# leotimus/binary-recommendation

Measured on AMD Instinct MI355X. Metric: (user,item) pairs/sec at batch 65536 dim 64, higher is better.
Workload: dtype f32; 1 GPU; NeuMF-A full training step (trainers/NFC_plain.py graph: 4 embeddings, 128->100->50->10->1, BCE, Keras-Adam adam_dense), embed_dim=64, 1000000 users x 100000 items per GPU, batch 65536 per GPU, uniform ids; global_batch=65536, parallelism=single GPU, steps_per_graph_launch=4, optimizer=adam_dense (deferred replay)

## Files before the change

### binary-recommendation_amd/csrc/dense_fwd.hip

```cpp
#include "common.h"
#include <stdlib.h>
#include "philox.h"
#include "dense.h"
#include "stamps.h"

namespace br {

using f32x4 = __attribute__((ext_vector_type(4))) float;

constexpr int kRep = BR_STAT_REPLICAS;
#ifdef BR_ABLATE_MFMA
#define BR_ABLATE_KEEP(c) (c)
#else
#define BR_ABLATE_KEEP(c) true
#endif

__device__ __forceinline__ f32x4 mfma16(float a, float b, f32x4 c) {
  return __builtin_amdgcn_mfma_f32_16x16x4f32(a, b, c, 0, 0, 0);
}


__global__ __launch_bounds__(256) void keep_bits_kernel(KeepArgs a) {
  dropout_resolve(a.drop);
  keep_bits_block(a, (int)blockIdx.y, (int64_t)blockIdx.x);
}

struct FwdArgs {
  const float* x; int64_t ldx;
  const float* W; const float* bias;
  float* y; int64_t ldy;
  int64_t batch;
  int K, N, act;
  const float* scale; const float* shift;
  brBnFold bn;
  const uint32_t* keep; int kw;
  float inv_keep;
  double* stats;
  const float* yin;
};

__device__ __forceinline__ float keep_if(float x, uint32_t w, uint32_t pos) {
  const int m = __builtin_amdgcn_sbfe((int)w, pos, 1u);
  return __int_as_float(__float_as_int(x) & m);
}

__device__ __forceinline__ float act_fwd(float z, int sigmask, float floor_) {
  const float s = __builtin_amdgcn_rcpf(1.0f + __builtin_amdgcn_exp2f(z * -1.44269504088896340736f));
  const float m = fmaxf(z, floor_);
  return __int_as_float((__float_as_int(s) & sigmask) | (__float_as_int(m) & ~sigmask));
}

template <int KJ, bool VEC>
__device__ __forceinline__ void fwd_load_tile(float4 (&av)[KJ], uint32_t (&kb)[(KJ + 1) / 2], const FwdArgs& a, int64_t tile, int c16, int g) {
  int64_t arow = (tile << 4) + c16;
  arow = arow < a.batch ? arow : a.batch - 1;
  const float* p = a.x + arow * a.ldx + 4 * g;
  const int klast = 16 * (KJ - 1) + 4 * g;
  if (VEC) {
#pragma unroll
    for (int j = 0; j < KJ - 1; ++j) av[j] = *reinterpret_cast<const float4*>(p + 16 * j);
    av[KJ - 1] = *reinterpret_cast<const float4*>(klast < a.K ? p + 16 * (KJ - 1) : p - 4 * g);
  } else {
#pragma unroll
    for (int j = 0; j < KJ - 1; ++j) av[j] = make_float4(p[16 * j], p[16 * j + 1], p[16 * j + 2], p[16 * j + 3]);
    const float* q = p - 4 * g;
    const int K1 = a.K - 1;
    av[KJ - 1] = make_float4(q[klast < K1 ? klast : K1], q[klast + 1 < K1 ? klast + 1 : K1], q[klast + 2 < K1 ? klast + 2 : K1], q[klast + 3 < K1 ? klast + 3 : K1]);
  }
  if (a.keep) {
    const uint32_t* kr = a.keep + arow * a.kw;
#pragma unroll
    for (int w = 0; w < (KJ + 1) / 2; ++w) kb[w] = kr[w];
  }
}

constexpr int kPatchLd = 20;

template <bool VEC>
__device__ __forceinline__ void fwd_epilogue(const f32x4& acc, const FwdArgs& a, float* patch, float* yrow, int64_t rbase, int nt, int c16, int g,
                                             const int (&vmask)[4], bool row_ok, float bv, int sigmask, float floor_, float& ssum, float& ssq) {
  const int n = nt * 16 + c16;
  const bool last = nt * 16 + 16 > a.N;
  const int cmask = (!last || n < a.N) ? -1 : 0;
  float yv[4] = {0.f, 0.f, 0.f, 0.f};
  if (a.yin) {
#pragma unroll
    for (int r = 0; r < 4; ++r) yv[r] = a.yin[(rbase + (vmask[r] ? 4 * g + r : 0)) * a.ldy + (cmask ? n : 0)];
  }
#pragma unroll
  for (int r = 0; r < 4; ++r) {
    const float z = fmaf(acc[r], a.inv_keep, bv) + yv[r];
    const float v = __int_as_float(__float_as_int(act_fwd(z, sigmask, floor_)) & vmask[r] & cmask);
    ssum += v;
    ssq = fmaf(v, v, ssq);
    patch[(4 * g + r) * kPatchLd + c16] = v;
  }
  __builtin_amdgcn_wave_barrier();
  const float4 o = *reinterpret_cast<const float4*>(patch + c16 * kPatchLd + 4 * g);
  __builtin_amdgcn_wave_barrier();
  float* dst = yrow + nt * 16;
  const int n0 = nt * 16 + 4 * g;
  if (VEC) {
    if (row_ok && (!last || n0 < a.N)) *reinterpret_cast<float4*>(dst) = o;
  } else if (row_ok) {
    if (n0 + 0 < a.N) dst[0] = o.x;
    if (n0 + 1 < a.N) dst[1] = o.y;
    if (n0 + 2 < a.N) dst[2] = o.z;
    if (n0 + 3 < a.N) dst[3] = o.w;
  }
}

template <bool VEC, int WN, int NT>
__device__ __forceinline__ void fwd_epilogue_multi(const f32x4 (&acc)[4], const FwdArgs& a, float* patch4, float* yrow, int64_t rbase, int nt0, int c16, int g,
                                                   const int (&vmask)[4], bool row_ok, const float* bs, int sigmask, float floor_, float (&ssum)[NT], float (&ssq)[NT]) {
#pragma unroll
  for (int w = 0; w < WN; ++w) {
    const int nt = nt0 + w, n = nt * 16 + c16;
    const bool last = nt * 16 + 16 > a.N;
    const int cmask = (!last || n < a.N) ? -1 : 0;
    const float bv = bs[n];
    float* patch = patch4 + w * 16 * kPatchLd;
#pragma unroll
    for (int r = 0; r < 4; ++r) {
      float z = fmaf(acc[w][r], a.inv_keep, bv);
      if (a.yin) z += a.yin[(rbase + (vmask[r] ? 4 * g + r : 0)) * a.ldy + (cmask ? n : 0)];
      const float v = __int_as_float(__float_as_int(act_fwd(z, sigmask, floor_)) & vmask[r] & cmask);
      ssum[nt] += v;
      ssq[nt] = fmaf(v, v, ssq[nt]);
      patch[(4 * g + r) * kPatchLd + c16] = v;
    }
  }
  __builtin_amdgcn_wave_barrier();
  const float* pr = patch4 + c16 * kPatchLd + 4 * g;
  const float4 z4 = make_float4(0.f, 0.f, 0.f, 0.f);
  const float4 o0 = *reinterpret_cast<const float4*>(pr);
  const float4 o1 = WN > 1 ? *reinterpret_cast<const float4*>(pr + 1 * 16 * kPatchLd) : z4;
  const float4 o2 = WN > 2 ? *reinterpret_cast<const float4*>(pr + 2 * 16 * kPatchLd) : z4;
  const float4 o3 = WN > 3 ? *reinterpret_cast<const float4*>(pr + 3 * 16 * kPatchLd) : z4;
  auto put = [&](const float4& o, int w) {
    const int nt = nt0 + w, n0 = nt * 16 + 4 * g;
    float* dst = yrow + nt * 16;
    if (VEC) {
      if (n0 < a.N) *reinterpret_cast<float4*>(dst) = o;
    } else {
      if (n0 + 0 < a.N) dst[0] = o.x;
      if (n0 + 1 < a.N) dst[1] = o.y;
      if (n0 + 2 < a.N) dst[2] = o.z;
      if (n0 + 3 < a.N) dst[3] = o.w;
    }
  };
  if (row_ok) {
    put(o0, 0);
    if (WN > 1) put(o1, 1);
    if (WN > 2) put(o2, 2);
    if (WN > 3) put(o3, 3);
  }
}

template <int NT, int KJ, bool VEC, int WPS, bool EMU>
__global__ __launch_bounds__(256 * WPS, WPS) void dense_fwd_kernel(const FwdArgs a) {
  extern __shared__ __attribute__((aligned(16))) float smem[];
  constexpr int kFwdThreads = 256 * WPS, kFwdWaves = 4 * WPS;
  constexpr int Np = NT * 16, Kp = KJ * 16, KWJ = (KJ + 1) / 2;
  constexpr int KB = (KJ + 1) / 2;
  constexpr int kWsFloats = EMU ? KB * 3 * 4 * Np * 4 : Kp * Np;
  float* Ws = smem;
  float* ssb = Ws + kWsFloats;
  float* bs = ssb + 2 * Kp;
  float* patches = bs + Np;
  constexpr int kPatchesPerWave = WPS == 2 ? 4 : 1;
  float* redw = patches + kFwdWaves * kPatchesPerWave * 16 * kPatchLd;
  const int lane = threadIdx.x & 63, wave = threadIdx.x >> 6;
  const int c16 = lane & 15, g = lane >> 4;
  const int K = a.K, N = a.N;
  const int64_t batch = a.batch;
  const int64_t n_tiles = (batch + 15) >> 4;
  const int64_t tstride = (int64_t)gridDim.x * kFwdWaves;
  {
    const int slot = __builtin_amdgcn_readfirstlane(wave >> 2);
    if (slot == 0) __builtin_amdgcn_s_setprio(3);
    else if (slot == 1) __builtin_amdgcn_s_setprio(2);
    else if (slot == 2) __builtin_amdgcn_s_setprio(1);
  }

  BR_STAMP_DECL;
  BR_STAMP_RT(10);
  BR_STAMP(0);
  const bool wquad = EMU && (N & 3) == 0;
  constexpr int NQ = Np / 4, TOTQ = KB * 4 * NQ, TRQ = EMU ? (TOTQ + kFwdThreads - 1) / kFwdThreads : 1;
  constexpr int TOTS = KB * 4 * Np, TRS = EMU ? (TOTS + kFwdThreads - 1) / kFwdThreads : 1;
  float4 wq[TRQ][8];
  float wv1[TRS][8];
  if constexpr (EMU) {
    if (wquad) {
#pragma unroll
      for (int i = 0; i < TRQ; ++i) {
        const int idx = threadIdx.x + i * kFwdThreads;
        const int idc = idx < TOTQ ? idx : 0;
        const int Jg = idc / NQ, n = (idc - Jg * NQ) * 4;
        const int J = Jg >> 2, gg = Jg & 3;
        const int nc = n < N ? n : 0;
#pragma unroll
        for (int q = 0; q < 8; ++q) {
          const int k = 32 * J + 16 * (q >> 2) + 4 * gg + (q & 3);
          wq[i][q] = *reinterpret_cast<const float4*>(a.W + (int64_t)(k < K ? k : 0) * N + nc);
        }
      }
    } else {
#pragma unroll
      for (int i = 0; i < TRS; ++i) {
        const int idx = threadIdx.x + i * kFwdThreads;
        const int idc = idx < TOTS ? idx : 0;
        const int Jg = idc / Np, n = idc - Jg * Np;
        const int J = Jg >> 2, gg = Jg & 3;
        const int nc = n < N ? n : N - 1;
#pragma unroll
        for (int q = 0; q < 8; ++q) {
          const int k = 32 * J + 16 * (q >> 2) + 4 * gg + (q & 3);
          wv1[i][q] = a.W[(k < K ? k : K - 1) * N + nc];
        }
      }
    }
  }
  float4 av[KJ];
  uint32_t kb[KWJ];
  int64_t tile = (int64_t)blockIdx.x * kFwdWaves + wave;
  fwd_load_tile<KJ, VEC>(av, kb, a, tile, c16, g);
  BR_STAMP(1);

  if (wquad) {
#pragma unroll
    for (int i = 0; i < TRQ; ++i) {
      const int idx = threadIdx.x + i * kFwdThreads;
      const int Jg = idx / NQ, n = (idx - Jg * NQ) * 4;
      const int J = Jg >> 2, gg = Jg & 3;
      const int nin = n < N ? -1 : 0;
      uint32_t* wsu = reinterpret_cast<uint32_t*>(Ws);
#pragma unroll
      for (int e = 0; e < 4; ++e) {
        uint32_t ph[4], pm[4], pl[4];
#pragma unroll
        for (int q = 0; q < 4; ++q) {
          const int k0 = 32 * J + 16 * (q >> 1) + 4 * gg + 2 * (q & 1);
          const float4 v0 = wq[i][2 * q], v1 = wq[i][2 * q + 1];
          const float f0 = e == 0 ? v0.x : (e == 1 ? v0.y : (e == 2 ? v0.z : v0.w)), f1 = e == 0 ? v1.x : (e == 1 ? v1.y : (e == 2 ? v1.z : v1.w));
          split3(__int_as_float(__float_as_int(f0) & nin & (k0 < K ? -1 : 0)), __int_as_float(__float_as_int(f1) & nin & (k0 + 1 < K ? -1 : 0)), ph[q], pm[q], pl[q]);
        }
        if (idx < TOTQ) {
          *reinterpret_cast<uint4*>(wsu + ((((J * 3 + 0) * 4 + gg) * Np + n + e) << 2)) = make_uint4(ph[0], ph[1], ph[2], ph[3]);
          *reinterpret_cast<uint4*>(wsu + ((((J * 3 + 1) * 4 + gg) * Np + n + e) << 2)) = make_uint4(pm[0], pm[1], pm[2], pm[3]);
          *reinterpret_cast<uint4*>(wsu + ((((J * 3 + 2) * 4 + gg) * Np + n + e) << 2)) = make_uint4(pl[0], pl[1], pl[2], pl[3]);
        }
      }
      __builtin_amdgcn_sched_barrier(0);
    }
  } else if constexpr (EMU) {
    constexpr int TOT = TOTS, TR = TRS;
    auto& wv = wv1;
#pragma unroll
    for (int i = 0; i < TR; ++i) {
      const int idx = threadIdx.x + i * kFwdThreads;
      const int Jg = idx / Np, n = idx - Jg * Np;
      const int J = Jg >> 2, gg = Jg & 3;
      uint32_t ph[4], pm[4], pl[4];
#pragma unroll
      for (int q = 0; q < 4; ++q) {
        const int k0 = 32 * J + 16 * (q >> 1) + 4 * gg + 2 * (q & 1);
        const float w0 = (n < N && k0 < K) ? wv[i][2 * q] : 0.f, w1 = (n < N && k0 + 1 < K) ? wv[i][2 * q + 1] : 0.f;
        split3(w0, w1, ph[q], pm[q], pl[q]);
      }
      if (idx < TOT) {
        uint32_t* wsu = reinterpret_cast<uint32_t*>(Ws);
        *reinterpret_cast<uint4*>(wsu + ((((J * 3 + 0) * 4 + gg) * Np + n) << 2)) = make_uint4(ph[0], ph[1], ph[2], ph[3]);
        *reinterpret_cast<uint4*>(wsu + ((((J * 3 + 1) * 4 + gg) * Np + n) << 2)) = make_uint4(pm[0], pm[1], pm[2], pm[3]);
        *reinterpret_cast<uint4*>(wsu + ((((J * 3 + 2) * 4 + gg) * Np + n) << 2)) = make_uint4(pl[0], pl[1], pl[2], pl[3]);
      }
      __builtin_amdgcn_sched_barrier(0);
    }
  } else
  {
    constexpr int TOT = KJ * 4 * Np, TR = (TOT + kFwdThreads - 1) / kFwdThreads;
    float wv[TR][4];
#pragma unroll
    for (int i = 0; i < TR; ++i) {
      const int idx = threadIdx.x + i * kFwdThreads;
      const int idc = idx < TOT ? idx : 0;
      const int jg = idc / Np, n = idc - jg * Np;
      const int k0 = 4 * jg;
      const int nc = n < N ? n : N - 1;
#pragma unroll
      for (int q = 0; q < 4; ++q) wv[i][q] = a.W[(k0 + q < K ? k0 + q : K - 1) * N + nc];
    }
#pragma unroll
    for (int i = 0; i < TR; ++i) {
      const int idx = threadIdx.x + i * kFwdThreads;
      const int jg = idx / Np, n = idx - jg * Np;
      const int k0 = 4 * jg;
      const bool nin = n < N;
      if (idx < TOT)
        *reinterpret_cast<float4*>(Ws + idx * 4) = make_float4((nin && k0 + 0 < K) ? wv[i][0] : 0.f, (nin && k0 + 1 < K) ? wv[i][1] : 0.f,
                                                                (nin && k0 + 2 < K) ? wv[i][2] : 0.f, (nin && k0 + 3 < K) ? wv[i][3] : 0.f);
    }
  }
  for (int k = threadIdx.x; k < Kp; k += kFwdThreads) {
    float sc = k < K ? 1.f : 0.f, sh = 0.f;
    if (k < K && a.bn.stats) {
      double s1 = 0.0, s2 = 0.0;
      for (int r = 0; r < kRep; ++r) { s1 += a.bn.stats[(size_t)r * 2 * K + k]; s2 += a.bn.stats[(size_t)r * 2 * K + K + k]; }
      const double mu = s1 / a.bn.batch_total;
      double var = s2 / a.bn.batch_total - mu * mu;
      if (var < 0.0) var = 0.0;
      const float muf = (float)mu, varf = (float)var;
      const float rs = 1.0f / sqrtf(varf + a.bn.eps);
      sc = a.bn.gamma[k] * rs;
      sh = a.bn.beta[k] - muf * sc;
      if (blockIdx.x == 0) {
        a.bn.scale[k] = sc; a.bn.shift[k] = sh; a.bn.mean[k] = muf; a.bn.rstd[k] = rs;
        if (a.bn.moving_mean) {
          a.bn.moving_mean[k] = a.bn.moving_mean[k] * a.bn.momentum + muf * (1.0f - a.bn.momentum);
          a.bn.moving_var[k] = a.bn.moving_var[k] * a.bn.momentum + varf * (1.0f - a.bn.momentum);
        }
      }
    } else if (k < K && a.scale) { sc = a.scale[k]; sh = a.shift[k]; }
    ssb[k] = sc;
    ssb[Kp + k] = sh;
  }
  for (int n = threadIdx.x; n < Np; n += kFwdThreads) bs[n] = (a.bias && n < N) ? a.bias[n] : 0.f;
  BR_STAMP(2);
  __syncthreads();
  BR_STAMP(3);

  float* patch = patches + wave * kPatchesPerWave * 16 * kPatchLd;
  float ssum[NT], ssq[NT];
#pragma unroll
  for (int nt = 0; nt < NT; ++nt) { ssum[nt] = 0.f; ssq[nt] = 0.f; }
  const int sigmask = a.act == BR_ACT_SIGMOID ? -1 : 0;
  const float floor_ = a.act == BR_ACT_RELU ? 0.f : -__builtin_inff();

  while (tile < n_tiles) {
    const int64_t rbase = tile << 4;
    const bool affine = a.scale || a.bn.stats || 16 * KJ != K;
    if (VEC && (K & 3)) {
      const int klast = 16 * (KJ - 1) + 4 * g;
      if (klast + 1 >= K) av[KJ - 1].y = 0.f;
      if (klast + 2 >= K) av[KJ - 1].z = 0.f;
      if (klast + 3 >= K) av[KJ - 1].w = 0.f;
    }
#pragma unroll
    for (int j = 0; j < KJ; ++j) {
      if (affine) {
        const int k = 16 * j + 4 * g;
        const float4 sc = *reinterpret_cast<const float4*>(ssb + k), sh = *reinterpret_cast<const float4*>(ssb + Kp + k);
        av[j].x = av[j].x * sc.x + sh.x; av[j].y = av[j].y * sc.y + sh.y; av[j].z = av[j].z * sc.z + sh.z; av[j].w = av[j].w * sc.w + sh.w;
      }
      if (a.keep) {
        const uint32_t w = kb[j >> 1], p0 = 16u * (j & 1) + 4u * g;
        av[j].x = keep_if(av[j].x, w, p0); av[j].y = keep_if(av[j].y, w, p0 + 1);
        av[j].z = keep_if(av[j].z, w, p0 + 2); av[j].w = keep_if(av[j].w, w, p0 + 3);
      }
      __builtin_amdgcn_sched_barrier(0);
    }
    BR_STAMP(4);
    const int64_t left = batch - rbase;
    const int rows_left16 = left > 16 ? 16 : (int)left;
    int vmask[4];
#pragma unroll
    for (int r = 0; r < 4; ++r) vmask[r] = (4 * g + r < rows_left16) ? -1 : 0;
    const bool row_ok = c16 < rows_left16;
    float* yrow = a.y + (rbase + (row_ok ? c16 : 0)) * a.ldy + 4 * g;
    float4 avn[WPS == 2 ? KJ : 1];
    uint32_t kbn[WPS == 2 ? KWJ : 1];
    const bool has_next = tile + tstride < n_tiles;
    if (WPS == 2 && has_next) fwd_load_tile<KJ, VEC>(reinterpret_cast<float4 (&)[KJ]>(avn), reinterpret_cast<uint32_t (&)[KWJ]>(kbn), a, tile + tstride, c16, g);
    constexpr bool PRESPLIT = EMU && WPS == 2;
    uint32_t ah[PRESPLIT ? KB : 1][4], am[PRESPLIT ? KB : 1][4], al[PRESPLIT ? KB : 1][4];
    auto split_block = [&](int J, uint32_t (&h)[4], uint32_t (&m)[4], uint32_t (&l)[4]) {
      const int j1 = 2 * J + 1 < KJ ? 2 * J + 1 : 0;
      split3(av[2 * J].x, av[2 * J].y, h[0], m[0], l[0]);
      split3(av[2 * J].z, av[2 * J].w, h[1], m[1], l[1]);
      if (2 * J + 1 < KJ) {
        split3(av[j1].x, av[j1].y, h[2], m[2], l[2]);
        split3(av[j1].z, av[j1].w, h[3], m[3], l[3]);
      } else {
        h[2] = h[3] = m[2] = m[3] = l[2] = l[3] = 0u;
      }
    };
    if constexpr (PRESPLIT) {
#pragma unroll
      for (int J = 0; J < KB; ++J) {
        split_block(J, ah[J], am[J], al[J]);
        __builtin_amdgcn_sched_barrier(0);
// ... 101 lines not shown
      }
    }
  }
  BR_STAMP(9);
  BR_STAMP_RT(11);
  BR_STAMP_FLUSH(blockIdx.x * kFwdWaves + wave);
}

}

using namespace br;

static inline int tiles16(int v) { return (v + 15) / 16; }
constexpr int kMaxT = 8;

extern "C" int64_t brDropoutKeepWords(int64_t batch, int K) { return (batch > 0 ? batch : 0) * (int64_t)((K + 31) / 32); }

extern "C" int brDropoutKeepBits(float drop_p, uint64_t seed, uint32_t step, int64_t row0, int64_t batch, int n_sites, const uint32_t* sites,
                                 const int* widths, uint32_t* const* out, brStream stream) {
  return br::dropout_keep_bits_ahead(drop_p, seed, step, 0, row0, batch, n_sites, sites, widths, out, stream);
}

int br::make_keep_args(KeepArgs& a, float drop_p, uint64_t seed, uint32_t step, uint32_t step_add, int64_t row0, int64_t batch, int n_sites,
                       const uint32_t* sites, const int* widths, uint32_t* const* out) {
  BR_CHECK_ARG(n_sites >= 1 && n_sites <= 3 && sites && widths && out && batch >= 0, "brDropoutKeepBits: bad args (1..3 sites)");
  BR_CHECK_ARG(drop_p > 0.f && drop_p < 1.f, "brDropoutKeepBits: drop_p must be in (0,1)");
  a.n_sites = n_sites;
  for (int i = 0; i < 3; ++i) {
    const int j = i < n_sites ? i : 0;
    BR_CHECK_ARG(widths[j] >= 1 && out[j], "brDropoutKeepBits: bad site %d", j);
    a.s[i].out = out[j]; a.s[i].K = widths[j]; a.s[i].kw = (widths[j] + 31) / 32; a.s[i].site = sites[j];
  }
  a.drop = make_dropout(drop_p, seed, step, 0);
  if (const StepStateDev* ss = current_step_state()) a.drop.step_ptr = &ss->step;
  a.drop.step_add = step_add;
  a.row0 = row0; a.batch = batch;
  return BR_OK;
}

int br::dropout_keep_bits_ahead(float drop_p, uint64_t seed, uint32_t step, uint32_t step_add, int64_t row0, int64_t batch, int n_sites,
                                const uint32_t* sites, const int* widths, uint32_t* const* out, brStream stream) {
  KeepArgs a;
  const int rc = make_keep_args(a, drop_p, seed, step, step_add, row0, batch, n_sites, sites, widths, out);
  if (rc != BR_OK) return rc;
  if (batch == 0) return BR_OK;
  int kwmax = 0;
  for (int i = 0; i < n_sites; ++i) kwmax = a.s[i].kw > kwmax ? a.s[i].kw : kwmax;
  const dim3 grid((unsigned)ceil_div(batch * kwmax, 256), (unsigned)n_sites);
  keep_bits_kernel<<<grid, 256, 0, (hipStream_t)stream>>>(a);
  BR_CHECK_LAUNCH("brDropoutKeepBits");
  return BR_OK;
}

template <int NT, int KJ, bool VEC, int WPS, bool EMU>
static void launch_fwd_v(unsigned grid, size_t shmem, hipStream_t s, const FwdArgs& a) {
  static bool attr_set = false;
  if (!attr_set) {
    (void)hipFuncSetAttribute((const void*)dense_fwd_kernel<NT, KJ, VEC, WPS, EMU>, hipFuncAttributeMaxDynamicSharedMemorySize, 150 * 1024);
    attr_set = true;
  }
  dense_fwd_kernel<NT, KJ, VEC, WPS, EMU><<<grid, 256 * WPS, shmem, s>>>(a);
}
static int fwd_wps(int64_t batch, bool vec, int KJ, int NT, bool emu) {
  static const int forced = [] { const char* e = getenv("BR_FWD_WPS"); return e ? atoi(e) : 0; }();
  if (!vec) return 4;
  if (forced == 2 || forced == 4) return forced;
  if (emu && KJ >= 5 && NT >= 3 && NT != 4) return 2;
  return (KJ >= 8 && ceil_div(batch, (int64_t)16) >= (int64_t)2 * 256 * 8) ? 2 : 4;
}

template <int NT, int KJ>
static void launch_fwd(size_t shmem_words_fixed, int Np, hipStream_t s, const FwdArgs& a, bool emu) {
  const bool vec = (a.ldx % 4 == 0) && ((reinterpret_cast<uintptr_t>(a.x) & 15) == 0) && (a.ldy % 4 == 0) && ((reinterpret_cast<uintptr_t>(a.y) & 15) == 0) &&
                   (a.yin == nullptr || a.K % 4 == 0);
  const int wps = fwd_wps(a.batch, vec, KJ, NT, emu);
  const int waves = 4 * wps;
  const size_t shmem = (shmem_words_fixed + (size_t)waves * (wps == 2 ? 4 : 1) * 16 * kPatchLd + (size_t)waves * 2 * Np) * sizeof(float);
  const int64_t wgs = ceil_div(ceil_div(a.batch, (int64_t)16), (int64_t)waves);
  const unsigned grid = (unsigned)(wgs < 1 ? 1 : (wgs > 256 ? 256 : wgs));
  if (emu) {
    if (vec && wps == 2) launch_fwd_v<NT, KJ, true, 2, true>(grid, shmem, s, a);
    else if (vec) launch_fwd_v<NT, KJ, true, 4, true>(grid, shmem, s, a);
    else launch_fwd_v<NT, KJ, false, 4, true>(grid, shmem, s, a);
    return;
  }
  if (vec && wps == 2) launch_fwd_v<NT, KJ, true, 2, false>(grid, shmem, s, a);
  else if (vec) launch_fwd_v<NT, KJ, true, 4, false>(grid, shmem, s, a);
  else launch_fwd_v<NT, KJ, false, 4, false>(grid, shmem, s, a);
}

static int dense_forward_one(FwdArgs a, hipStream_t s) {
  const int NT = tiles16(a.N), KJ = tiles16(a.K), Kp = KJ * 16, Np = NT * 16;
  const bool emu = br::mlp_bf16x6();
  const size_t wimg = emu ? (size_t)((KJ + 1) / 2) * 3 * 4 * Np * 4 : (size_t)Kp * Np;
  const size_t fixed = wimg + 2 * (size_t)Kp + (size_t)Np;
#define BR_FWD_KJ(NTv, KJv) case KJv: launch_fwd<NTv, KJv>(fixed, Np, s, a, emu); break;
#define BR_FWD(NTv)                                                                                        \
  case NTv:                                                                                                \
    switch (KJ) { BR_FWD_KJ(NTv, 1) BR_FWD_KJ(NTv, 2) BR_FWD_KJ(NTv, 3) BR_FWD_KJ(NTv, 4) BR_FWD_KJ(NTv, 5) \
                  BR_FWD_KJ(NTv, 6) BR_FWD_KJ(NTv, 7) BR_FWD_KJ(NTv, 8) default: break; }                  \
    break;
  switch (NT) {
    BR_FWD(1) BR_FWD(2) BR_FWD(3) BR_FWD(4) BR_FWD(5) BR_FWD(6) BR_FWD(7) BR_FWD(8)
    default: br::set_error("brDenseForward: unsupported N"); return BR_ERR_UNSUPPORTED;
  }
  BR_CHECK_LAUNCH("brDenseForward");
  return BR_OK;
}

static inline int split_k(int K) { return ((K / 2 + 31) / 32) * 32; }

extern "C" int brDenseForward(const float* x, int64_t ldx, const float* W, const float* bias, float* y, int64_t ldy,
                              int64_t batch, int K, int N, int act, const float* in_scale, const float* in_shift,
                              const brBnFold* in_bn, float drop_p, const uint32_t* keep, double* stats, brStream stream) {
  BR_CHECK_ARG(x && W && y && batch >= 0 && K >= 1 && N >= 1, "brDenseForward: bad args");
  BR_CHECK_ARG(K <= 2 * kMaxT * 16 && N <= kMaxT * 16, "brDenseForward: K=%d N=%d exceed %d / %d", K, N, 2 * kMaxT * 16, kMaxT * 16);
  BR_CHECK_ARG(ldx >= K && ldy >= N, "brDenseForward: bad leading dims");
  BR_CHECK_ARG((in_scale == nullptr) == (in_shift == nullptr), "brDenseForward: in_scale/in_shift both or neither");
  BR_CHECK_ARG(!in_bn || (!in_scale && in_bn->stats && in_bn->gamma && in_bn->beta && in_bn->scale && in_bn->shift && in_bn->mean && in_bn->rstd &&
                          in_bn->batch_total > 0 && (in_bn->moving_mean == nullptr) == (in_bn->moving_var == nullptr) && K <= kMaxT * 16),
               "brDenseForward: in_bn needs stats, gamma, beta and the four outputs, no in_scale/in_shift, K <= %d", kMaxT * 16);
  BR_CHECK_ARG(drop_p >= 0.f && drop_p < 1.f, "brDenseForward: drop_p out of [0,1)");
  BR_CHECK_ARG((drop_p > 0.f) == (keep != nullptr), "brDenseForward: keep bits (brDropoutKeepBits) are required exactly when drop_p > 0");
  if (batch == 0) return BR_OK;
  hipStream_t s = (hipStream_t)stream;
  const int kw = (K + 31) / 32;
  brBnFold nofold{};
  FwdArgs a{x, ldx, W, bias, y, ldy, batch, K, N, act, in_scale, in_shift, in_bn ? *in_bn : nofold, keep, kw, drop_p > 0.f ? 1.0f / (1.0f - drop_p) : 1.0f, stats, nullptr};
  if (K <= kMaxT * 16) return dense_forward_one(a, s);
  const int Ka = split_k(K);
  FwdArgs h = a;
  h.K = Ka; h.bias = nullptr; h.act = BR_ACT_LINEAR; h.stats = nullptr;
  int rc = dense_forward_one(h, s);
  if (rc != BR_OK) return rc;
  h = a;
  h.x = x + Ka; h.W = W + (int64_t)Ka * N; h.K = K - Ka; h.yin = y;
  if (in_scale) { h.scale = in_scale + Ka; h.shift = in_shift + Ka; }
  if (keep) h.keep = keep + Ka / 32;
  return dense_forward_one(h, s);
}
```

### binary-recommendation_amd/ops.py

```python
from __future__ import annotations

import ctypes

import torch

from . import _lib
from ._lib import check

I32, I64 = 0, 1
ACT = {"linear": 0, "sigmoid": 1, "relu": 2}
LOSS = {"bce": 0, "mse": 1}
STAT_REPLICAS = 8


_RAW_STREAM = getattr(torch._C, "_cuda_getCurrentRawStream", None)
_DEV_INDEX = None


def _stream() -> int:
    global _DEV_INDEX
    if _RAW_STREAM is None:
        return torch.cuda.current_stream().cuda_stream
    if _DEV_INDEX is None:
        _DEV_INDEX = torch.cuda.current_device()
# ... 336 lines not shown
                                 _stream()), "brAdamFlat")


def adagrad_rows_sorted(table, acc, index: RowIndex, row_grads, ldg, lr, eps=1e-7):
    check(_lib.load().brAdagradRowsSorted(_f32(table, "table").data_ptr(), _f32(acc, "acc").data_ptr(), table.shape[0],
                                          table.shape[1], index.sorted_ids.data_ptr(), index.id_type,
                                          index.sorted_pos.data_ptr(), index.n, row_grads.data_ptr(), int(ldg), float(lr),
                                          float(eps), index.seg_ws(table.shape[1]).data_ptr(), _stream()), "brAdagradRowsSorted")


def adagrad_flat(theta, acc, g, lr, eps=1e-7):
    check(_lib.load().brAdagradFlat(_f32(theta, "theta").data_ptr(), _f32(acc, "acc").data_ptr(), _f32(g, "g").data_ptr(),
                                    theta.numel(), float(lr), float(eps), _stream()), "brAdagradFlat")


REPLAY = {"exact": 0, "fast": 1}


def new_step_state(device, beta1=0.9, beta2=0.999, eps=1e-7, replay="fast") -> torch.Tensor:
    st = torch.zeros(int(_lib.load().brStepStateBytes()) // 4, dtype=torch.int32, device=device)
    check(_lib.load().brStepStateInit(st.data_ptr(), float(beta1), float(beta2), float(eps), REPLAY[replay], _stream()), "brStepStateInit")
    return st


def adam_alpha(lr: float, t: int, beta1=0.9, beta2=0.999) -> float:
    return lr * (1.0 - beta2 ** t) ** 0.5 / (1.0 - beta1 ** t)


def dropout_keep_words(batch, K) -> int:
    return int(_lib.load().brDropoutKeepWords(batch, K))


def dropout_keep_bits(drop_p, seed, step, row0, batch, sites, widths, outs=None):
    n = len(sites)
    if outs is None:
        dev = torch.device("cuda", torch.cuda.current_device())
        outs = [torch.empty(dropout_keep_words(batch, k), dtype=torch.int32, device=dev) for k in widths]
    S = (ctypes.c_uint32 * n)(*[int(s) for s in sites])
    Wd = (ctypes.c_int * n)(*[int(k) for k in widths])
    OP = (ctypes.c_void_p * n)(*[o.data_ptr() for o in outs])
    check(_lib.load().brDropoutKeepBits(float(drop_p), int(seed), int(step), int(row0), int(batch), n, S, Wd, OP, _stream()), "brDropoutKeepBits")
    return outs


def dense_forward(x, W, bias, y, act, in_scale=None, in_shift=None, drop_p=0.0, seed=0, step=0, site=0, row0=0,
                  stats=None, batch=None, keep=None):
    B = x.shape[0] if batch is None else batch
    K, N = W.shape
    if drop_p > 0 and keep is None and B > 0:
        keep = dropout_keep_bits(drop_p, seed, step, row0, B, [site], [K])[0]
    check(_lib.load().brDenseForward(x.data_ptr(), x.stride(0), _f32(W, "W").data_ptr(), _p(bias), y.data_ptr(), y.stride(0),
                                     B, K, N, ACT[act], _p(in_scale), _p(in_shift), None, float(drop_p), _p(keep) if drop_p > 0 else 0,
                                     _p(stats), _stream()), "brDenseForward")


def bn_finalize(stats, batch_total, gamma, beta, eps, momentum, moving_mean, moving_var, scale, shift, mean, rstd):
    check(_lib.load().brBnFinalize(stats.data_ptr(), float(batch_total), gamma.data_ptr(), beta.data_ptr(), float(eps),
                                   float(momentum), _p(moving_mean), _p(moving_var), scale.data_ptr(), shift.data_ptr(),
                                   mean.data_ptr(), rstd.data_ptr(), gamma.numel(), _stream()), "brBnFinalize")


def bn_inference(gamma, beta, moving_mean, moving_var, eps, scale, shift):
    check(_lib.load().brBnInference(gamma.data_ptr(), beta.data_ptr(), moving_mean.data_ptr(), moving_var.data_ptr(),
                                    float(eps), scale.data_ptr(), shift.data_ptr(), gamma.numel(), _stream()), "brBnInference")


def dense_backward_slabs(batch, K, N) -> int:
    return int(_lib.load().brDenseBackwardSlabs(batch, K, N))


def dense_backward_ws_floats(batch, K, N) -> int:
    return int(_lib.load().brDenseBackwardWorkspaceFloats(batch, K, N))


def dense_backward(gy, y, x, W, act, slabs, n_slabs, gx=None, out_bn=None, bn_sums=None, batch_total=None,
                   in_scale=None, in_shift=None, in_bn=None, in_drop_p=0.0, in_site=0, seed=0, step=0, row0=0,
                   in_bn_sums=None, batch=None, dz_ws=None, keep=None):
    B = gy.shape[0] if batch is None else batch
    K, N = W.shape
    om, ors, og = out_bn if out_bn is not None else (None, None, None)
    im, irs = in_bn if in_bn is not None else (None, None)
    if dz_ws is None:
        dz_ws = torch.empty(dense_backward_ws_floats(B, K, N), dtype=torch.float32, device=gy.device)
    if in_drop_p > 0 and keep is None and B > 0:
        keep = dropout_keep_bits(in_drop_p, seed, step, row0, B, [in_site], [K])[0]
    check(_lib.load().brDenseBackward(gy.data_ptr(), gy.stride(0), y.data_ptr(), y.stride(0), x.data_ptr(), x.stride(0),
                                      W.data_ptr(), B, K, N, ACT[act], _p(om), _p(ors), _p(og), _p(bn_sums),
                                      float(batch_total if batch_total is not None else B), _p(in_scale), _p(in_shift),
                                      _p(im), _p(irs), float(in_drop_p), _p(keep) if in_drop_p > 0 else 0,
                                      _p(gx), gx.stride(0) if gx is not None else 0, dz_ws.data_ptr(), slabs.data_ptr(), int(n_slabs),
                                      _p(in_bn_sums), _stream()), "brDenseBackward")


def reduce_slabs(slabs, n_slabs, slab_elems, out):
    check(_lib.load().brReduceSlabs(slabs.data_ptr(), int(n_slabs), int(slab_elems), out.data_ptr(), _stream()), "brReduceSlabs")


def bn_param_grads(bn_sums, dgamma, dbeta):
    check(_lib.load().brBnParamGrads(bn_sums.data_ptr(), dgamma.data_ptr(), dbeta.data_ptr(), dgamma.numel(), _stream()),
          "brBnParamGrads")


def bn_param_grads_pair(bn_sums_a, dgamma_a, dbeta_a, bn_sums_b, dgamma_b, dbeta_b):
    check(_lib.load().brBnParamGradsPair(bn_sums_a.data_ptr(), dgamma_a.data_ptr(), dbeta_a.data_ptr(), dgamma_a.numel(),
                                         bn_sums_b.data_ptr(), dgamma_b.data_ptr(), dbeta_b.data_ptr(), dgamma_b.numel(), _stream()),
          "brBnParamGradsPair")
# ... 864 lines not shown
```

### include/binrec.h

```cpp
#ifndef BINREC_H
#define BINREC_H
#include <stdint.h>

#ifdef __cplusplus
extern "C" {
#endif

typedef void* brStream;

enum { BR_OK = 0, BR_ERR_ARG = -1, BR_ERR_HIP = -2, BR_ERR_UNSUPPORTED = -3, BR_ERR_WORKSPACE = -4 };
enum { BR_IDS_I32 = 0, BR_IDS_I64 = 1 };
enum { BR_ACT_LINEAR = 0, BR_ACT_SIGMOID = 1, BR_ACT_RELU = 2 };
enum { BR_LOSS_BCE = 0, BR_LOSS_MSE = 1 };
enum { BR_MAX_TABLES = 8, BR_SUM_SLOTS = 64, BR_STAT_REPLICAS = 8, BR_METRIC_SUMS = 8 };

const char* brGetLastError(void);
int brVersion(void);
int brDeviceInfo(int* cu_count, int* wave_size, char* arch, int arch_len);

int brGatherRows(int n_tables, const float* const* tables, const int64_t* table_rows,
                 const void* const* ids, float* const* outs, int dim, int64_t batch,
                 int id_type, int* err_flag, brStream stream);

int brRowDot(const float* a, const float* b, float* out, int dim, int64_t batch, brStream stream);
// ... 56 lines not shown
                           void* sorted_ids_b, int32_t* sorted_pos_b, int id_type, int64_t n, int64_t seg_len, int64_t seg_stride, int64_t seg_off_a,
                           int64_t seg_off_b, int* err_flag, brStream stream);
int brGatherRowsDeferredPairSeg(const float* table_a, const float* m_a, const float* v_a, const int32_t* last_a, int64_t rows_a, const float* table_b,
                                const float* m_b, const float* v_b, const int32_t* last_b, int64_t rows_b, const void* ids, float* out, int dim,
                                int id_type, int64_t n, int64_t seg_len, int64_t seg_stride, int64_t seg_off_a, int64_t seg_off_b,
                                const void* step_state, double beta1, double beta2, double eps, int64_t ld_out, int* err_flag, brStream stream);
int brGatherRowsPairSeg(const float* table_a, int64_t rows_a, const float* table_b, int64_t rows_b, const void* ids, float* out, int dim, int id_type,
                        int64_t n, int64_t seg_len, int64_t seg_stride, int64_t seg_off_a, int64_t seg_off_b, int64_t ld_out, int* err_flag,
                        brStream stream);
int brRowsToSlotsPair(const float* src_a, const float* src_b, int64_t ld, const int32_t* bpos_a, const int32_t* bpos_b, float* dst_a,
                      float* dst_b, int64_t n_slots, int dim, brStream stream);
int64_t brSegmentScratchFloats(int64_t n, int dim);
int brSegmentSumRows(const void* sorted_ids, int id_type, const int32_t* sorted_pos, int64_t n,
                     const float* row_grads, int64_t ldg, int dim, float* out_rows,
                     int32_t* head_flag, float* seg_ws, brStream stream);
int brScatterAddRows(float* g_table, int64_t table_rows, const void* ids, int id_type,
                     int64_t n, const float* rows, int dim, int* err_flag, brStream stream);

int brAdamRowsSorted(float* table, float* m, float* v, int64_t table_rows, int dim,
                     const void* sorted_ids, int id_type, const int32_t* sorted_pos, int64_t n,
                     const float* row_grads, int64_t ldg, const float* row_grads_hi,
                     int64_t ldg_hi, int split, double alpha_t, double beta1, double beta2,
                     double eps, uint8_t* mark, float* seg_ws, brStream stream);
int brAdamDenseSweep(float* table, float* m, float* v, int64_t table_rows, int dim,
                     double alpha_t, double beta1, double beta2, double eps, uint8_t* mark,
                     brStream stream);
int brAdamFlat(float* theta, float* m, float* v, const float* g, int64_t n, double alpha_t,
               double beta1, double beta2, double eps, brStream stream);

int brAdagradRowsSorted(float* table, float* acc, int64_t table_rows, int dim,
                        const void* sorted_ids, int id_type, const int32_t* sorted_pos, int64_t n,
                        const float* row_grads, int64_t ldg, double lr, double eps,
                        float* seg_ws, brStream stream);
int brAdagradFlat(float* theta, float* acc, const float* g, int64_t n, double lr, double eps,
                  brStream stream);

int64_t brDropoutKeepWords(int64_t batch, int K);
int brDropoutKeepBits(float drop_p, uint64_t seed, uint32_t step, int64_t row0, int64_t batch, int n_sites,
                      const uint32_t* sites, const int* widths, uint32_t* const* out, brStream stream);

typedef struct brBnFold {
  const double* stats;
  double batch_total;
  const float* gamma; const float* beta;
  float eps; float momentum;
  float* moving_mean; float* moving_var;
  float* scale; float* shift; float* mean; float* rstd;
} brBnFold;

int brDenseForward(const float* x, int64_t ldx, const float* W, const float* bias, float* y,
                   int64_t ldy, int64_t batch, int K, int N, int act, const float* in_scale,
                   const float* in_shift, const brBnFold* in_bn, float drop_p, const uint32_t* keep,
                   double* stats, brStream stream);
int brBnFinalize(const double* stats, double batch_total, const float* gamma, const float* beta,
                 float eps, float momentum, float* moving_mean, float* moving_var, float* scale,
                 float* shift, float* mean, float* rstd, int N, brStream stream);
int brBnInference(const float* gamma, const float* beta, const float* moving_mean,
                  const float* moving_var, float eps, float* scale, float* shift, int N,
                  brStream stream);
int brDenseBackwardSlabs(int64_t batch, int K, int N);
int64_t brDenseBackwardWorkspaceFloats(int64_t batch, int K, int N);
int brDenseBackward(const float* gy, int64_t ldgy, const float* y, int64_t ldy, const float* x,
                    int64_t ldx, const float* W, int64_t batch, int K, int N, int act,
                    const float* out_mean, const float* out_rstd, const float* out_gamma,
                    const double* bn_sums, double batch_total, const float* in_scale,
                    const float* in_shift, const float* in_mean, const float* in_rstd,
                    float in_drop_p, const uint32_t* keep, float* gx, int64_t ldgx, float* dz_ws,
                    float* dW_slabs, int n_slabs, double* in_bn_sums, brStream stream);
int brBnParamGrads(const double* bn_sums, float* dgamma, float* dbeta, int N, brStream stream);
int brBnParamGradsPair(const double* sums_a, float* dgamma_a, float* dbeta_a, int Na, const double* sums_b, float* dgamma_b,
                       float* dbeta_b, int Nb, brStream stream);
int brReduceSlabs(const float* slabs, int n_slabs, int64_t slab_elems, float* out, brStream stream);

int brDenseFinalize(const float* const* slabs, const int* n_slabs, const int64_t* slab_elems, const int64_t* grad_off,
                    const double* const* bn_sums, const int* bn_n, const int64_t* dgamma_off, const int64_t* dbeta_off,
                    float* theta, float* m, float* v, float* grad, int64_t n, double alpha_t, double beta1, double beta2,
                    double eps, brStream stream);

int brNeumfTailSlabs(int64_t batch);
int64_t brNeumfTailSlabElems(int n2, int n3);
int brNeumfTailFused(const float* a2, int64_t lda2, const float* W3, const float* b3, const float* w4, const float* b4,
                     const float* dot, const float* labels, const float* scale2, const float* shift2, const float* mean2,
                     const float* rstd2, const brBnFold* bn2, float drop_p, const uint32_t* keep,
                     int64_t batch, int n2, int n3, int act, int mf_first, int loss, float inv_batch, float* a3,
                     float* logit, float* prob, double* sums, float* ddot, float* gh2, int64_t ldgh2, double* bn_sums,
                     float* slabs, int n_slabs, brStream stream);

int brHeadSlabs(int64_t batch);
int brNeumfHead(const float* a3, int64_t lda3, const float* dot, const float* labels,
                const float* w4, const float* b4, int64_t batch, int N3, int mf_first, int loss,
                float inv_batch, float* logit, float* prob, double* sums, float* da3,
                int64_t ldda3, float* ddot, float* head_slabs, int n_slabs, brStream stream);

int brBceLogits(const float* z, const float* y, int64_t batch, float inv_batch, float* prob,
                float* dz, double* sums, brStream stream);

int64_t brInBatchSoftmaxWorkspaceBytes(int64_t Bq, int64_t Bc, int dim);
int brInBatchSoftmaxLse(const float* Q, const float* C, const void* q_pos_ids,
                        const void* cand_ids, int id_type, int64_t Bq, int64_t Bc, int dim,
                        int64_t diag_offset, float* row_lse, double* loss_sum, void* ws,
                        int64_t ws_bytes, brStream stream);
int brInBatchSoftmaxLseGradQ(const float* Q, const float* C, const void* q_pos_ids,
                             const void* cand_ids, int id_type, int64_t Bq, int64_t Bc, int dim,
                             int64_t diag_offset, float* row_lse, double* loss_sum, float* dQ,
                             void* ws, int64_t ws_bytes, brStream stream);
int brInBatchSoftmaxGrad(const float* Q, const float* C, const void* q_pos_ids,
// ... 258 lines not shown
```

Measured before the change: 224.8 million pairs/s.

## Add k-block streaming forward path for bf16x6 dense kernel with prefetch

Adds a STREAM variant of the dense forward kernel, enabled by default for the emulated (bf16x6) vectorized case. It issues the activation tile loads and the BN/bias parameter loads early so they overlap the weight staging. Inside the k-loop it double-buffers weight fragment reads from LDS across MFMA groups, and it can prefetch the next tile or process two tiles at once. The aim is to hide global and LDS latency in the forward GEMMs, at the cost of extra register pressure and a more complex code path.

```diff
diff --git a/binary-recommendation_amd/csrc/dense_fwd.hip b/binary-recommendation_amd/csrc/dense_fwd.hip
--- a/binary-recommendation_amd/csrc/dense_fwd.hip
+++ b/binary-recommendation_amd/csrc/dense_fwd.hip
@@ -1,5 +1,6 @@
 #include "common.h"
 #include <stdlib.h>
+#include <type_traits>
 #include "philox.h"
 #include "dense.h"
 #include "stamps.h"
@@ -71,6 +72,34 @@
     const uint32_t* kr = a.keep + arow * a.kw;
 #pragma unroll
     for (int w = 0; w < (KJ + 1) / 2; ++w) kb[w] = kr[w];
+  }
+}
+
+template <int KJ, int R>
+__device__ __forceinline__ void fwd_load_stream(float4 (&av)[R][KJ], uint32_t (&kb)[R][(KJ + 1) / 2], const FwdArgs& a, int64_t tile, int64_t tstride, int c16, int g) {
+  const float* p[R];
+  int64_t arow[R];
+#pragma unroll
+  for (int r = 0; r < R; ++r) {
+    arow[r] = ((tile + r * tstride) << 4) + c16;
+    arow[r] = arow[r] < a.batch ? arow[r] : a.batch - 1;
+    p[r] = a.x + arow[r] * a.ldx + 4 * g;
+  }
+  if (a.keep) {
+#pragma unroll
+    for (int r = 0; r < R; ++r) {
+      const uint32_t* kr = a.keep + arow[r] * a.kw;
+#pragma unroll
+      for (int w = 0; w < (KJ + 1) / 2; ++w) kb[r][w] = kr[w];
+    }
+  }
+  const int klast = 16 * (KJ - 1) + 4 * g;
+#pragma unroll
+  for (int j = 0; j < KJ; ++j) {
+#pragma unroll
+    for (int r = 0; r < R; ++r)
+      av[r][j] = *reinterpret_cast<const float4*>(j < KJ - 1 ? p[r] + 16 * j : (klast < a.K ? p[r] + 16 * (KJ - 1) : p[r] - 4 * g));
+    __builtin_amdgcn_sched_barrier(0);
   }
 }
 
@@ -157,8 +186,9 @@
   }
 }
 
-template <int NT, int KJ, bool VEC, int WPS, bool EMU>
+template <int NT, int KJ, bool VEC, int WPS, bool EMU, bool STREAM = false, bool PAIR = false>
 __global__ __launch_bounds__(256 * WPS, WPS) void dense_fwd_kernel(const FwdArgs a) {
+  static_assert(!STREAM || (EMU && VEC), "the k-block-ordered form exists for the bf16x6 VEC instantiations");
   extern __shared__ __attribute__((aligned(16))) float smem[];
   constexpr int kFwdThreads = 256 * WPS, kFwdWaves = 4 * WPS;
   constexpr int Np = NT * 16, Kp = KJ * 16, KWJ = (KJ + 1) / 2;
@@ -186,6 +216,21 @@
   BR_STAMP_DECL;
   BR_STAMP_RT(10);
   BR_STAMP(0);
+  const int tk = threadIdx.x;
+  float e_sc, e_sh, e_bias, e_gamma, e_beta, e_mm, e_mv;
+  double e_s1[kRep], e_s2[kRep];
+  if constexpr (STREAM) {
+    static_assert(KJ * 16 <= 256 * WPS && NT * 16 <= 256 * WPS, "one staging thread per column");
+    if (tk < K) {
+      if (a.bn.stats) {
+#pragma unroll
+        for (int r = 0; r < kRep; ++r) { e_s1[r] = a.bn.stats[(size_t)r * 2 * K + tk]; e_s2[r] = a.bn.stats[(size_t)r * 2 * K + K + tk]; }
+        e_gamma = a.bn.gamma[tk]; e_beta = a.bn.beta[tk];
+        if (blockIdx.x == 0 && a.bn.moving_mean) { e_mm = a.bn.moving_mean[tk]; e_mv = a.bn.moving_var[tk]; }
+      } else if (a.scale) { e_sc = a.scale[tk]; e_sh = a.shift[tk]; }
+    }
+    if (a.bias && tk < N) e_bias = a.bias[tk];
+  }
   const bool wquad = EMU && (N & 3) == 0;
   constexpr int NQ = Np / 4, TOTQ = KB * 4 * NQ, TRQ = EMU ? (TOTQ + kFwdThreads - 1) / kFwdThreads : 1;
   constexpr int TOTS = KB * 4 * Np, TRS = EMU ? (TOTS + kFwdThreads - 1) / kFwdThreads : 1;
@@ -225,8 +270,43 @@
   float4 av[KJ];
   uint32_t kb[KWJ];
   int64_t tile = (int64_t)blockIdx.x * kFwdWaves + wave;
-  fwd_load_tile<KJ, VEC>(av, kb, a, tile, c16, g);
+  constexpr int R2 = (STREAM && WPS == 2 && PAIR) ? 2 : 1;
+  constexpr int NS = (STREAM && WPS == 2) ? 2 : 1;
+  float4 avs[NS][KJ];
+  uint32_t kbs[NS][KWJ];
+  if constexpr (STREAM) {
+    tile = (int64_t)blockIdx.x * kFwdWaves + __builtin_amdgcn_readfirstlane(wave);
+    fwd_load_stream<KJ, R2>(reinterpret_cast<float4 (&)[R2][KJ]>(avs), reinterpret_cast<uint32_t (&)[R2][KWJ]>(kbs), a, tile, tstride, c16, g);
+  } else
+    fwd_load_tile<KJ, VEC>(av, kb, a, tile, c16, g);
   BR_STAMP(1);
+  if constexpr (STREAM) {
+    if (tk < Kp) {
+      float sc = tk < K ? 1.f : 0.f, sh = 0.f;
+      if (tk < K && a.bn.stats) {
+        double s1 = 0.0, s2 = 0.0;
+#pragma unroll
+        for (int r = 0; r < kRep; ++r) { s1 += e_s1[r]; s2 += e_s2[r]; }
+        const double mu = s1 / a.bn.batch_total;
+        double var = s2 / a.bn.batch_total - mu * mu;
+        if (var < 0.0) var = 0.0;
+        const float muf = (float)mu, varf = (float)var;
+        const float rs = 1.0f / sqrtf(varf + a.bn.eps);
+        sc = e_gamma * rs;
+        sh = e_beta - muf * sc;
+        if (blockIdx.x == 0) {
+          a.bn.scale[tk] = sc; a.bn.shift[tk] = sh; a.bn.mean[tk] = muf; a.bn.rstd[tk] = rs;
+          if (a.bn.moving_mean) {
+            a.bn.moving_mean[tk] = e_mm * a.bn.momentum + muf * (1.0f - a.bn.momentum);
+            a.bn.moving_var[tk] = e_mv * a.bn.momentum + varf * (1.0f - a.bn.momentum);
+          }
+        }
+      } else if (tk < K && a.scale) { sc = e_sc; sh = e_sh; }
+      ssb[tk] = sc;
+      ssb[Kp + tk] = sh;
+    }
+    if (tk < Np) bs[tk] = (a.bias && tk < N) ? e_bias : 0.f;
+  }
 
   if (wquad) {
 #pragma unroll
@@ -302,6 +382,7 @@
                                                                 (nin && k0 + 2 < K) ? wv[i][2] : 0.f, (nin && k0 + 3 < K) ? wv[i][3] : 0.f);
     }
   }
+  if constexpr (!STREAM) {
   for (int k = threadIdx.x; k < Kp; k += kFwdThreads) {
     float sc = k < K ? 1.f : 0.f, sh = 0.f;
     if (k < K && a.bn.stats) {
@@ -326,6 +407,7 @@
     ssb[Kp + k] = sh;
   }
   for (int n = threadIdx.x; n < Np; n += kFwdThreads) bs[n] = (a.bias && n < N) ? a.bias[n] : 0.f;
+  }
   BR_STAMP(2);
   __syncthreads();
   BR_STAMP(3);
@@ -337,6 +419,146 @@
   const int sigmask = a.act == BR_ACT_SIGMOID ? -1 : 0;
   const float floor_ = a.act == BR_ACT_RELU ? 0.f : -__builtin_inff();
 
+  if constexpr (STREAM) {
+    const bool affine = a.scale || a.bn.stats || 16 * KJ != K;
+    const float* wl_ = Ws + ((g * Np + c16) << 2);
+    auto stream_tiles = [&](auto RC, auto SC) {
+      constexpr int R = decltype(RC)::value, S = decltype(SC)::value;
+      int64_t rbase[R];
+      int vmask[R][4];
+      bool row_ok[R];
+      float* yrow[R];
+#pragma unroll
+      for (int r = 0; r < R; ++r) {
+        rbase[r] = (tile + r * tstride) << 4;
+        const int64_t left = batch - rbase[r];
+        const int rows_left16 = left > 16 ? 16 : (int)left;
+#pragma unroll
+        for (int q = 0; q < 4; ++q) vmask[r][q] = (4 * g + q < rows_left16) ? -1 : 0;
+        row_ok[r] = c16 < rows_left16;
+        yrow[r] = a.y + (rbase[r] + (row_ok[r] ? c16 : 0)) * a.ldy + 4 * g;
+      }
+      f32x4 acc[R][NT];
+      const f32x4 zero4 = (f32x4){0.f, 0.f, 0.f, 0.f};
+      float4 bq[2][3];
+#pragma unroll
+      for (int p = 0; p < 3; ++p) bq[0][p] = *reinterpret_cast<const float4*>(wl_ + ((p * 4 * Np) << 2));
+#pragma unroll
+      for (int J = 0; J < KB; ++J) {
+        uint32_t th[R][4], tm[R][4], tl[R][4];
+#pragma unroll
+        for (int jj = 0; jj < 2; ++jj) {
+          const int j = 2 * J + jj;
+          if (j < KJ) {
+            float4 sc = make_float4(1.f, 1.f, 1.f, 1.f), sh = make_float4(0.f, 0.f, 0.f, 0.f);
+            if (affine) { sc = *reinterpret_cast<const float4*>(ssb + 16 * j + 4 * g); sh = *reinterpret_cast<const float4*>(ssb + Kp + 16 * j + 4 * g); }
+#pragma unroll
+            for (int r = 0; r < R; ++r) {
+              float4& v = avs[S + r][j];
+              if (j == KJ - 1 && (K & 3)) {
+                const int klast = 16 * (KJ - 1) + 4 * g;
+                if (klast + 1 >= K) v.y = 0.f;
+                if (klast + 2 >= K) v.z = 0.f;
+                if (klast + 3 >= K) v.w = 0.f;
+              }
+              if (affine) { v.x = v.x * sc.x + sh.x; v.y = v.y * sc.y + sh.y; v.z = v.z * sc.z + sh.z; v.w = v.w * sc.w + sh.w; }
+              if (a.keep) {
+                const uint32_t w = kbs[S + r][J], p0 = 16u * jj + 4u * g;
+                v.x = keep_if(v.x, w, p0); v.y = keep_if(v.y, w, p0 + 1);
+                v.z = keep_if(v.z, w, p0 + 2); v.w = keep_if(v.w, w, p0 + 3);
+              }
+            }
+          }
+        }
+#pragma unroll
+        for (int r = 0; r < R; ++r) {
+          split3(avs[S + r][2 * J].x, avs[S + r][2 * J].y, th[r][0], tm[r][0], tl[r][0]);
+          split3(avs[S + r][2 * J].z, avs[S + r][2 * J].w, th[r][1], tm[r][1], tl[r][1]);
+          if (2 * J + 1 < KJ) {
+            constexpr int kj1 = KJ - 1;
+            const int j1 = 2 * J + 1 < KJ ? 2 * J + 1 : kj1;
+            split3(avs[S + r][j1].x, avs[S + r][j1].y, th[r][2], tm[r][2], tl[r][2]);
+            split3(avs[S + r][j1].z, avs[S + r][j1].w, th[r][3], tm[r][3], tl[r][3]);
+          } else {
+            th[r][2] = th[r][3] = tm[r][2] = tm[r][3] = tl[r][2] = tl[r][3] = 0u;
+          }
+        }
+        __builtin_amdgcn_sched_barrier(0);
+        if (J == 0) BR_STAMP(4);
+        bf16x8 xh[R], xm[R], xl[R];
+#pragma unroll
+        for (int r = 0; r < R; ++r) { xh[r] = frag8(th[r]); xm[r] = frag8(tm[r]); xl[r] = frag8(tl[r]); }
+#pragma unroll
+        for (int w = 0; w < NT; ++w) {
+          const int st = J * NT + w, cur = st & 1;
+          const int Jn = (w + 1 < NT) ? J : J + 1, wn = (w + 1 < NT) ? w + 1 : 0;
+          if (Jn < KB) {
+#pragma unroll
+            for (int p = 0; p < 3; ++p) bq[cur ^ 1][p] = *reinterpret_cast<const float4*>(wl_ + (((Jn * 3 + p) * 4 * Np + wn * 16) << 2));
+          }
+          const bf16x8 wh = frag8(bq[cur][0]), wm = frag8(bq[cur][1]), wl = frag8(bq[cur][2]);
+#pragma unroll
+          for (int r = 0; r < R; ++r) acc[r][w] = mfma_bf16(xl[r], wh, J == 0 ? zero4 : acc[r][w]);
+#pragma unroll
+          for (int r = 0; r < R; ++r) acc[r][w] = mfma_bf16(xh[r], wl, acc[r][w]);
+#pragma unroll
+          for (int r = 0; r < R; ++r) acc[r][w] = mfma_bf16(xm[r], wm, acc[r][w]);
+#pragma unroll
+          for (int r = 0; r < R; ++r) acc[r][w] = mfma_bf16(xm[r], wh, acc[r][w]);
+#pragma unroll
+          for (int r = 0; r < R; ++r) acc[r][w] = mfma_bf16(xh[r], wm, acc[r][w]);
+#pragma unroll
+          for (int r = 0; r < R; ++r) acc[r][w] = mfma_bf16(xh[r], wh, acc[r][w]);
+          __builtin_amdgcn_sched_barrier(0);
+        }
+      }
+      BR_STAMP(5);
+#pragma unroll
+      for (int r = 0; r < R; ++r) {
+#pragma unroll
+        for (int nt0 = 0; nt0 < NT; nt0 += 4) {
+          const int Wn = (NT - nt0) < 4 ? (NT - nt0) : 4;
+          if constexpr (WPS == 2) {
+            f32x4 a4[4];
+#pragma unroll
+            for (int w = 0; w < 4; ++w) a4[w] = acc[r][nt0 + w < NT ? nt0 + w : NT - 1];
+            if (Wn == 4) fwd_epilogue_multi<VEC, 4, NT>(a4, a, patch, yrow[r], rbase[r], nt0, c16, g, vmask[r], row_ok[r], bs, sigmask, floor_, ssum, ssq);
+            else if (Wn == 3) fwd_epilogue_multi<VEC, 3, NT>(a4, a, patch, yrow[r], rbase[r], nt0, c16, g, vmask[r], row_ok[r], bs, sigmask, floor_, ssum, ssq);
+            else if (Wn == 2) fwd_epilogue_multi<VEC, 2, NT>(a4, a, patch, yrow[r], rbase[r], nt0, c16, g, vmask[r], row_ok[r], bs, sigmask, floor_, ssum, ssq);
+            else fwd_epilogue_multi<VEC, 1, NT>(a4, a, patch, yrow[r], rbase[r], nt0, c16, g, vmask[r], row_ok[r], bs, sigmask, floor_, ssum, ssq);
+            __builtin_amdgcn_sched_barrier(0);
+          } else {
+#pragma unroll
+            for (int w = 0; w < 4; ++w) {
+              if (w < Wn) {
+                const float bv = bs[(nt0 + w) * 16 + c16];
+                fwd_epilogue<VEC>(acc[r][nt0 + w], a, patch, yrow[r], rbase[r], nt0 + w, c16, g, vmask[r], row_ok[r], bv, sigmask, floor_, ssum[nt0 + w], ssq[nt0 + w]);
+                __builtin_amdgcn_sched_barrier(0);
+              }
+            }
+          }
+        }
+        BR_STAMP(6 + r);
+      }
+      if (R == 1) BR_STAMP(7);
+    };
+    using I0 = std::integral_constant<int, 0>; using I1 = std::integral_constant<int, 1>; using I2 = std::integral_constant<int, 2>;
+    if constexpr (R2 == 2) {
+      if (tile + tstride < n_tiles) { stream_tiles(I2{}, I0{}); tile += 2 * tstride; }
+      else if (tile < n_tiles) { stream_tiles(I1{}, I0{}); tile += tstride; }
+    } else if constexpr (NS == 2) {
+      const bool second = tile + tstride < n_tiles;
+      if (second) fwd_load_stream<KJ, 1>(reinterpret_cast<float4 (&)[1][KJ]>(avs[1]), reinterpret_cast<uint32_t (&)[1][KWJ]>(kbs[1]), a, tile + tstride, tstride, c16, g);
+      if (tile < n_tiles) { stream_tiles(I1{}, I0{}); tile += tstride; }
+      if (second) { stream_tiles(I1{}, I1{}); tile += tstride; }
+    } else if (tile < n_tiles) { stream_tiles(I1{}, I0{}); tile += tstride; }
+    while (tile < n_tiles) {
+      fwd_load_stream<KJ, 1>(reinterpret_cast<float4 (&)[1][KJ]>(avs), reinterpret_cast<uint32_t (&)[1][KWJ]>(kbs), a, tile, tstride, c16, g);
+      stream_tiles(I1{}, I0{});
+      tile += tstride;
+    }
+    BR_STAMP(8);
+  } else
   while (tile < n_tiles) {
     const int64_t rbase = tile << 4;
     const bool affine = a.scale || a.bn.stats || 16 * KJ != K;
@@ -544,14 +766,21 @@
   return BR_OK;
 }
 
-template <int NT, int KJ, bool VEC, int WPS, bool EMU>
+static int g_fwd_last_form = BR_FWD_FORM_NONE;
+
+template <int NT, int KJ, bool VEC, int WPS, bool EMU, bool STREAM = false, bool PAIR = false>
 static void launch_fwd_v(unsigned grid, size_t shmem, hipStream_t s, const FwdArgs& a) {
   static bool attr_set = false;
   if (!attr_set) {
-    (void)hipFuncSetAttribute((const void*)dense_fwd_kernel<NT, KJ, VEC, WPS, EMU>, hipFuncAttributeMaxDynamicSharedMemorySize, 150 * 1024);
+    (void)hipFuncSetAttribute((const void*)dense_fwd_kernel<NT, KJ, VEC, WPS, EMU, STREAM, PAIR>, hipFuncAttributeMaxDynamicSharedMemorySize, 150 * 1024);
     attr_set = true;
   }
-  dense_fwd_kernel<NT, KJ, VEC, WPS, EMU><<<grid, 256 * WPS, shmem, s>>>(a);
+  dense_fwd_kernel<NT, KJ, VEC, WPS, EMU, STREAM, PAIR><<<grid, 256 * WPS, shmem, s>>>(a);
+  g_fwd_last_form = STREAM ? BR_FWD_FORM_STREAM : BR_FWD_FORM_PASSES;
+}
+static bool fwd_stream_enabled() {
+  const char* e = getenv("BR_FWD_STREAM");
+  return !(e && e[0] == '0');
 }
 static int fwd_wps(int64_t batch, bool vec, int KJ, int NT, bool emu) {
   static const int forced = [] { const char* e = getenv("BR_FWD_WPS"); return e ? atoi(e) : 0; }();
@@ -570,6 +799,13 @@
   const size_t shmem = (shmem_words_fixed + (size_t)waves * (wps == 2 ? 4 : 1) * 16 * kPatchLd + (size_t)waves * 2 * Np) * sizeof(float);
   const int64_t wgs = ceil_div(ceil_div(a.batch, (int64_t)16), (int64_t)waves);
   const unsigned grid = (unsigned)(wgs < 1 ? 1 : (wgs > 256 ? 256 : wgs));
+  if (emu && vec && fwd_stream_enabled()) {
+    static const bool pair = [] { const char* e = getenv("BR_FWD_PAIR"); return e && e[0] == '1'; }();
+    if (wps == 2 && pair) launch_fwd_v<NT, KJ, true, 2, true, true, true>(grid, shmem, s, a);
+    else if (wps == 2) launch_fwd_v<NT, KJ, true, 2, true, true>(grid, shmem, s, a);
+    else launch_fwd_v<NT, KJ, true, 4, true, true>(grid, shmem, s, a);
+    return;
+  }
   if (emu) {
     if (vec && wps == 2) launch_fwd_v<NT, KJ, true, 2, true>(grid, shmem, s, a);
     else if (vec) launch_fwd_v<NT, KJ, true, 4, true>(grid, shmem, s, a);
@@ -601,6 +837,8 @@
 }
 
 static inline int split_k(int K) { return ((K / 2 + 31) / 32) * 32; }
+
+extern "C" int brDenseForwardLastForm(void) { return g_fwd_last_form; }
 
 extern "C" int brDenseForward(const float* x, int64_t ldx, const float* W, const float* bias, float* y, int64_t ldy,
                               int64_t batch, int K, int N, int act, const float* in_scale, const float* in_shift,
diff --git a/binary-recommendation_amd/ops.py b/binary-recommendation_amd/ops.py
--- a/binary-recommendation_amd/ops.py
+++ b/binary-recommendation_amd/ops.py
@@ -412,6 +412,13 @@
     check(_lib.load().brDenseForward(x.data_ptr(), x.stride(0), _f32(W, "W").data_ptr(), _p(bias), y.data_ptr(), y.stride(0),
                                      B, K, N, ACT[act], _p(in_scale), _p(in_shift), None, float(drop_p), _p(keep) if drop_p > 0 else 0,
                                      _p(stats), _stream()), "brDenseForward")
+
+
+FWD_FORMS = {0: "none", 1: "passes", 2: "stream"}
+
+
+def dense_forward_last_form() -> str:
+    return FWD_FORMS[int(_lib.load().brDenseForwardLastForm())]
 
 
 def bn_finalize(stats, batch_total, gamma, beta, eps, momentum, moving_mean, moving_var, scale, shift, mean, rstd):
diff --git a/include/binrec.h b/include/binrec.h
--- a/include/binrec.h
+++ b/include/binrec.h
@@ -132,6 +132,8 @@
                    int64_t ldy, int64_t batch, int K, int N, int act, const float* in_scale,
                    const float* in_shift, const brBnFold* in_bn, float drop_p, const uint32_t* keep,
                    double* stats, brStream stream);
+enum { BR_FWD_FORM_NONE = 0, BR_FWD_FORM_PASSES = 1, BR_FWD_FORM_STREAM = 2 };
+int brDenseForwardLastForm(void);
 int brBnFinalize(const double* stats, double batch_total, const float* gamma, const float* beta,
                  float eps, float momentum, float* moving_mean, float* moving_var, float* scale,
                  float* shift, float* mean, float* rstd, int N, brStream stream);
```

Result: no change. 224.6 million pairs/s (median of 3 runs) (-0.1%).
